# HAHHHD/mllp

Hardware: AMD Instinct MI355X
Metric: LP instances/sec (fwd+bwd) on Netlib batch; achieved HBM GB/s on CSR SpMM (higher is better)
Workload: dtype f32; 1 GPU; netlib_full: BASELINE.json configs[2], 97 instances / 1,074,147 nnz per global batch, one block-diagonal batch per GPU, one Adam step per global batch: fwd + BCE + bwd + gradient all-reduce + Adam, fp32; global_batch=97, instances_rank0=97, nnz_rank0=1074147, hip_graph=False, parallelism=dp1

## Files before the change

mllp_amd/csrc/fused_kernels.hip:

```cpp
#include <algorithm>
#include <vector>

#include "device_utils.h"
#include "host_graph.h"
#include "internal.h"
#include "node_bodies.h"

namespace mllp {

typedef float f32x4m __attribute__((ext_vector_type(4)));

#ifdef MLLP_TIMING_BUILD
static int g_fused_abl = [] {
    const char* e = getenv("MLLP_FUSED_ABL");
    return e ? atoi(e) : 0;
}();
#define FUSED_ABL(bit) ((J.abl & (bit)) != 0)
__device__ unsigned long long g_fused_stamps[8192 * 8];
__device__ unsigned long long g_fused_stamps1[8192 * 8];
#define FUSED_STAMP(k)                                                                      \
    {                                                                                       \
        __builtin_amdgcn_sched_barrier(0);                                                  \
        const unsigned long long now_ = __builtin_amdgcn_s_memtime();                       \
        __builtin_amdgcn_sched_barrier(0);                                                  \
        stamp_sum[k] += now_ - stamp_last;                                                  \
        stamp_last = now_;                                                                  \
    }
#else
#define FUSED_ABL(bit) false
#define FUSED_STAMP(k)
#endif

constexpr int FT = 768;
constexpr int FW = FT / 64;
constexpr int RT = 1024;
constexpr int MAXJOBS = 2;

constexpr int NP = FUSED_NP;
static_assert(NP == FUSED_PARTS, "partition count");

struct PartTiers {
    int row0, n_block, n_wave, n_group, n_base;
};
struct ItemsDev {
    const int* __restrict__ sptr;
    const int2* __restrict__ sent;
    const float2* __restrict__ sax;
    int n_dst, nnz;
    const int* __restrict__ order;
    int nw, L;
    PartTiers part[NP];
};

static ItemsDev items_dev(const FusedOrient& o, int which) {
    const bool scalar = which == 1;
    ItemsDev d;
    d.order = which == 0 ? o.lst16 : which == 1 ? o.lst1 : o.lst16x2;
    d.nw = which == 0 ? o.nw16 : which == 1 ? o.nw1 : o.nw16x2;
    d.L = which == 0 ? o.L16 : which == 1 ? o.L1 : o.L16x2;
    d.sptr = o.sptr;
    d.sent = reinterpret_cast<const int2*>(o.sent);
    d.sax = reinterpret_cast<const float2*>(o.sax);
    d.n_dst = o.n_dst;
    d.nnz = o.nnz;
    for (int q = 0; q < NP; ++q) {
        const FusedTiersDev& t = scalar ? o.t1[q] : o.t16[q];
        d.part[q].row0 = o.row0[q];
        d.part[q].n_block = t.n_block; d.part[q].n_wave = t.n_wave; d.part[q].n_group = t.n_group; d.part[q].n_base = t.n_base;
    }
    return d;
}

constexpr int TS = 17;
constexpr int TILE = 16 * TS;
__device__ __forceinline__ void tile_put(float* tile, const float4& v, int lane) {
    float* d = tile + (lane >> 2) * TS + 4 * (lane & 3);
    d[0] = v.x; d[1] = v.y; d[2] = v.z; d[3] = v.w;
}
__device__ __forceinline__ float4 tile_get(const float* tile, int lane) {
    const float* d = tile + (lane >> 2) * TS + 4 * (lane & 3);
    return make_float4(d[0], d[1], d[2], d[3]);
}
__device__ __forceinline__ void tile_rows(const float* tile, int lane, float (&a)[4]) {
#pragma unroll
    for (int s = 0; s < 4; ++s) a[s] = tile[(lane & 15) * TS + 4 * s + (lane >> 4)];
}
__device__ __forceinline__ void tile_cols(const float* tile, int lane, float (&a)[4]) {
#pragma unroll
    for (int s = 0; s < 4; ++s) a[s] = tile[(4 * s + (lane >> 4)) * TS + (lane & 15)];
}
__device__ __forceinline__ void tile_put_result(float* tile, const f32x4m& d, int lane) {
#pragma unroll
    for (int j = 0; j < 4; ++j) tile[(4 * (lane >> 4) + j) * TS + (lane & 15)] = d[j];
}
struct MatB {
    float w[4];
};
__device__ __forceinline__ MatB matB(const float* __restrict__ W, int ld, int lane) {
    MatB b;
#pragma unroll
    for (int s = 0; s < 4; ++s) b.w[s] = W[(lane & 15) * ld + 4 * s + (lane >> 4)];
    return b;
}
__device__ __forceinline__ MatB matB_t(const float* __restrict__ W, int ld, int lane) {
    MatB b;
#pragma unroll
    for (int s = 0; s < 4; ++s) b.w[s] = W[(4 * s + (lane >> 4)) * ld + (lane & 15)];
    return b;
}
__device__ __forceinline__ void matB_store(float* lds, const MatB& b, int lane) {
    *reinterpret_cast<float4*>(lds + 4 * lane) = make_float4(b.w[0], b.w[1], b.w[2], b.w[3]);
}
__device__ __forceinline__ MatB matB_lds(const float* lds, int lane) {
    const float4 v = *reinterpret_cast<const float4*>(lds + 4 * lane);
    MatB b;
    b.w[0] = v.x; b.w[1] = v.y; b.w[2] = v.z; b.w[3] = v.w;
    return b;
}
__device__ __forceinline__ f32x4m mat_apply(const float (&a)[4], const MatB& b, f32x4m acc) {
// ... 646 lines not shown
            const float Sr = __shfl(S, row_l, 64), ur = __shfl(un, row_l, 64), zr = __shfl(zn, row_l, 64), xr = __shfl(x, row_l, 64);
            float4 v = lds4(W.bs + ch);
            fma4(Sr, lds4(W.bv + ch), v);
            fma4(ur, lds4(W.we + ch), v);
            fma4(zr, lds4(W.wv + ch), v);
            fma4(xr, lds4(W.ws + ch), v);
            if (row_l < n_valid)
                *reinterpret_cast<float4*>(J.h + (size_t)(base_row + row_l) * 16 + ch) =
                    make_float4(fmaxf(v.x, 0.0f), fmaxf(v.y, 0.0f), fmaxf(v.z, 0.0f), fmaxf(v.w, 0.0f));
        }
        if (r.writer) {
            J.Z[r.row] = zn;
            reinterpret_cast<float4*>(J.aux)[r.row] = make_float4(un, st.L > 0.0f ? st.m : 0.0f, rinv, S);
        }
        return;
    }
    if (!r.writer) return;
    float o[16];
#pragma unroll
    for (int c = 0; c < 16; ++c) {
        float v = W.bs[c];
        v = fmaf(S, W.bv[c], v);
        v = fmaf(un, W.we[c], v);
        v = fmaf(W.wv[c], zn, v);
        v = fmaf(W.ws[c], x, v);
        o[c] = fmaxf(v, 0.0f);
    }
    float4* hd = reinterpret_cast<float4*>(J.h + (size_t)r.row * 16);
    hd[0] = make_float4(o[0], o[1], o[2], o[3]);
    hd[1] = make_float4(o[4], o[5], o[6], o[7]);
    hd[2] = make_float4(o[8], o[9], o[10], o[11]);
    hd[3] = make_float4(o[12], o[13], o[14], o[15]);
    J.Z[r.row] = zn;
    reinterpret_cast<float4*>(J.aux)[r.row] = make_float4(un, st.L > 0.0f ? st.m : 0.0f, rinv, S);
}

__global__ __launch_bounds__(FT) void fused_fwd1_kernel(FwdLaunch1 A) {
    __shared__ FwdW1 Ws_[MAXJOBS];
    __shared__ float merge_lds[FW * 4];
    const int tid = threadIdx.x, lane = tid & 63;
    for (int j = 0; j < A.n_jobs; ++j) {
        const FwdJob1& J = A.job[j];
        FwdW1& W = Ws_[j];
        if (tid < 16) {
            W.wv[tid] = J.p.Wv[tid]; W.ws[tid] = J.p.Ws[tid];
            W.bv[tid] = J.p.bv[tid]; W.we[tid] = J.p.we[tid]; W.bs[tid] = J.p.bs[tid];
        }
        if (tid == 0) {
            W.pq = J.D[OFF_PQ]; W.pq0 = J.D[OFF_PQ0]; W.pt = J.D[OFF_PT]; W.pt0 = J.D[OFF_PT0];
        }
    }
    __syncthreads();
    const BlockPart B = block_part();
    for (int j = 0; j < A.n_jobs; ++j) {
        const FwdJob1& J = A.job[j];
        const PartTiers P = J.s.part[B.px];
        for (int k = B.bi; k < P.n_block; k += B.gp)
            fwd1_row(J, Ws_[j], block_slot<1>(J.s, P.row0 + k, tid), lane, merge_lds);
        WaveList wl = wave_list(J.s, B.px, B.gw);
        for (int c0 = 0; c0 < wl.L; c0 += 64) {
            wave_list_chunk(wl, c0, lane);
            int it = wave_list_get(wl, 0);
            SlotReq q = item_request<1>(J.s, P, max(it, 0), lane);
            for (int k = 0; it >= 0; ++k) {
                const int itn = wave_list_get(wl, k + 1);
                const RowSlot r = slot_make(q);
                q = item_request<1>(J.s, P, max(itn, 0), lane);
                fwd1_row(J, Ws_[j], r, lane, merge_lds);
                it = itn;
            }
        }
    }
}

struct BwdJob16 {
    ItemsDev s;
    const float* __restrict__ x_src;
    const float* __restrict__ x_dst;
    const float* __restrict__ D;
    ConvParams p;
    const float* __restrict__ h;
    const float* __restrict__ dh_a;
    const float* __restrict__ dh_b;
    const float* __restrict__ Z;
    const float* __restrict__ aux;
    float* __restrict__ rec;
    float* __restrict__ dx_dst;
    int mask_dx;
    float* __restrict__ stats;
#ifdef MLLP_TIMING_BUILD
    int abl;
#endif
};
struct BwdLaunch16 {
    BwdJob16 job[MAXJOBS];
    int n_jobs;
};
struct BwdW16 {
    float BWvT[256], BPq[256], BWsT[256], BPqT[256];
    float pq0[16], Pt[16], Pb[16], bv[16], we[16];
    float pt0;
};
struct BwdState {
    float4 dq;
    float ds, dt;
};

__device__ __forceinline__ void bwd16_step(const Gather4& g, int k0, int n_mine, const float4& qp, const float4& gv, float t,
                                           float m, float rinv, float ge, float cc, BwdState& st) {
#define MLLP_BWD_SLOT(K, A_, X_)                                                           \
    {                                                                                      \
        const float l_ = fmaf(A_, t, quad_sum(dot4(qp, X_)));                              \
        const float al_ = (k0 + K < n_mine) ? exp_acc(l_ - m) * rinv : 0.0f;               \
        const float dl_ = al_ * (quad_sum(dot4(gv, X_)) + fmaf(A_, ge, cc));               \
        st.ds += dl_;                                                                      \
        st.dt = fmaf(dl_, A_, st.dt);                                                      \
        fma4(dl_, X_, st.dq);                                                              \
    }
    MLLP_BWD_SLOT(0, g.a0, g.x0)
    MLLP_BWD_SLOT(1, g.a1, g.x1)
    MLLP_BWD_SLOT(2, g.a2, g.x2)
    MLLP_BWD_SLOT(3, g.a3, g.x3)
#undef MLLP_BWD_SLOT
}

// ... 317 lines not shown
    if (!dst16_merge<1>(bs, r.mode, merge_lds, tiles, lane, part)) return;
    dst16_dx(W, tiles, bs, r, JJ.dx_dst, true, xpos, part, lane);
    StatCols c;
    dst16_stat_cols(tiles, bs, r, false, part, lane, c);
    stats_accumulate(c, acc, park, lane);
}

__global__ __launch_bounds__(FT) void fused_l3_kernel(L3Job JJ) {
    __shared__ L3W W;
    __shared__ float merge_lds[FW * 20];
    __shared__ float head_lds[FW * 18];
    __shared__ float tiles_[FW * TB_N * TILE];
    __shared__ __attribute__((aligned(16))) float park_[FW * L3_PARK];
    const int tid = threadIdx.x, lane = tid & 63, wave = tid >> 6, part = lane & 3;
    const FwdJob16& J = JJ.f;
    stage_weights<true, true>(W, J.D, J.p, J.fcw, J.fcb, tid);
    __syncthreads();
    float* tiles = tiles_ + wave * TB_N * TILE;
    HeadAcc ha;
    ha.w = f4zero(); ha.b = 0.0f; ha.l = 0.0f;
    float* park = park_ + wave * L3_PARK;
    f32x4m acc[L3_REG_TILES];
#pragma unroll
    for (int i = 0; i < L3_REG_TILES; ++i) acc[i] = splat4(0.0f);
#pragma unroll
    for (int i = L3_REG_TILES; i < STAT_TILES; ++i) park_put(park, i - L3_REG_TILES, lane, splat4(0.0f));
    const BlockPart B = block_part();
    const PartTiers P = J.s.part[B.px];
    walk_two_deep(J, P, B, tid, [&](const RowSlot& r, const float4& xd, int2& en, int lrow, const SlotReq& q1, int it2,
                                    FwdNext& nx) __attribute__((always_inline)) {
        l3_row(JJ, W, P, r, xd, en, lrow, q1, it2, nx, part, lane, merge_lds, tiles, park, ha, acc);
    });
    __syncthreads();
#pragma unroll
    for (int i = 0; i < STAT_TILES; ++i) {
        const f32x4m a = i < L3_REG_TILES ? acc[min(i, L3_REG_TILES - 1)] : park_get(park, max(i - L3_REG_TILES, 0), lane);
        stats_tile_store(a, i, tiles_, JJ.stats, tid);
    }
    head_partials_store<FW>(ha, head_lds, J.head_part, tid);
}

struct SrcJob16 {
    ItemsDev s;
    const float* __restrict__ x;
    const float* __restrict__ rec;
    float* __restrict__ dx;
    const float* __restrict__ addp;
    float addw;
    int mask;
};
struct SrcLaunch16 {
    SrcJob16 job[MAXJOBS];
    int n_jobs;
};

__device__ __forceinline__ void src16_row(const SrcJob16& J, const RowSlot& r, float4& xj_io, int2& en, const SlotReq& qn,
                                          RowSlot& rn, int part, int lane, float* merge_lds) {
    const int n_mine = slot_count(r);
    const float4 xj = xj_io;
    const float4 addv = ld4(J.addp + (size_t)max(r.row, 0) * 16 + 4 * part);
    float4 acc = f4zero();
    for (int k0 = 0; __any(k0 < n_mine); k0 += 2) {
        const int colm = en.x;
        const float am = __int_as_float(en.y);
        const int c0 = quad_bcast_i<0>(colm), c1 = quad_bcast_i<1>(colm);
        const float a0 = quad_bcast<0>(am), a1 = quad_bcast<1>(am);
        const bool ok0 = k0 < n_mine, ok1 = k0 + 1 < n_mine;
        const float* rr0 = J.rec + (size_t)c0 * REC_W;
        const float* rr1 = J.rec + (size_t)c1 * REC_W;
        const float4 q0 = ld4(rr0 + 4 * part), g0 = ld4(rr0 + 16 + 4 * part), s0 = ld4(rr0 + 32);
        const float cc0 = rr0[36];
        const float4 q1 = ld4(rr1 + 4 * part), g1 = ld4(rr1 + 16 + 4 * part), s1 = ld4(rr1 + 32);
        const float cc1 = rr1[36];
        const int kn = k0 + 2 + (part & 1);
        en = kn < n_mine ? J.s.sent[r.first + kn * r.stride] : make_int2(0, 0);
        {
            const float l = fmaf(a0, s0.x, quad_sum(dot4(q0, xj)));
            const float al = ok0 ? exp_acc(l - s0.y) * s0.z : 0.0f;
            const float dl = al * (quad_sum(dot4(g0, xj)) + fmaf(a0, s0.w, cc0));
            fma4(al, g0, acc);
            fma4(dl, q0, acc);
        }
        {
            const float l = fmaf(a1, s1.x, quad_sum(dot4(q1, xj)));
            const float al = ok1 ? exp_acc(l - s1.y) * s1.z : 0.0f;
            const float dl = al * (quad_sum(dot4(g1, xj)) + fmaf(a1, s1.w, cc1));
            fma4(al, g1, acc);
            fma4(dl, q1, acc);
        }
    }
    rn = slot_make(qn);
    xj_io = rn.row >= 0 ? ld4(J.x + (size_t)rn.row * 16 + 4 * part) : f4zero();
    en = first_entries<2>(J.s, rn, part);
    if (r.mode >= 1) {
        acc.x = shared_sum4(acc.x, r.mode); acc.y = shared_sum4(acc.y, r.mode);
        acc.z = shared_sum4(acc.z, r.mode); acc.w = shared_sum4(acc.w, r.mode);
    }
    if (r.mode == 3) {
        const int wave = threadIdx.x >> 6;
        if (lane < 4) *reinterpret_cast<float4*>(merge_lds + wave * 20 + 4 * part) = acc;
        __syncthreads();
        float4 v = f4zero();
        for (int w = 0; w < FW; ++w) v = f4add(v, lds4(merge_lds + w * 20 + 4 * part));
        acc = v;
        __syncthreads();
    }
    fma4(J.addw, addv, acc);
    if (J.mask) {
        if (!(xj.x > 0.0f)) acc.x = 0.0f;
        if (!(xj.y > 0.0f)) acc.y = 0.0f;
        if (!(xj.z > 0.0f)) acc.z = 0.0f;
        if (!(xj.w > 0.0f)) acc.w = 0.0f;
    }
    if (r.writer) *reinterpret_cast<float4*>(J.dx + (size_t)r.row * 16 + 4 * part) = acc;
}

__global__ __launch_bounds__(FT) void fused_src16_kernel(SrcLaunch16 A) {
    __shared__ float merge_lds[FW * 20];
    const int tid = threadIdx.x, lane = tid & 63, part = lane & 3;
    const BlockPart B = block_part();
    for (int j = 0; j < A.n_jobs; ++j) {
        const SrcJob16& J = A.job[j];
        const PartTiers P = J.s.part[B.px];
        const RowSlot none = empty_slot();
        for (int k = B.bi; k < P.n_block; k += B.gp) {
            const RowSlot r = block_slot<4>(J.s, P.row0 + k, tid);
            float4 xj = ld4(J.x + (size_t)r.row * 16 + 4 * part);
            int2 en = first_entries<2>(J.s, r, part);
            RowSlot rn;
            src16_row(J, r, xj, en, empty_request(), rn, part, lane, merge_lds);
        }
        WaveList wl = wave_list(J.s, B.px, B.gw);
        for (int c0 = 0; c0 < wl.L; c0 += 64) {
            wave_list_chunk(wl, c0, lane);
            int it = wave_list_get(wl, 0);
            RowSlot r = it >= 0 ? item_slot<4>(J.s, P, it, lane) : none;
            float4 xj = r.row >= 0 ? ld4(J.x + (size_t)r.row * 16 + 4 * part) : f4zero();
            int2 en = first_entries<2>(J.s, r, part);
            for (int k = 0; it >= 0; ++k) {
                const int itn = wave_list_get(wl, k + 1);
                const SlotReq qn = itn >= 0 ? item_request<4>(J.s, P, itn, lane) : empty_request();
                RowSlot rn;
                src16_row(J, r, xj, en, qn, rn, part, lane, merge_lds);
                r = rn;
                it = itn;
            }
        }
    }
}

struct BwdJob1 {
    ItemsDev s;
    const float* __restrict__ x_dst;
    const float* __restrict__ D;
    ConvParams p;
    const float* __restrict__ g;
    const float* __restrict__ Z;
    const float* __restrict__ aux;
    float* __restrict__ stats;
};
struct BwdLaunch1 {
    BwdJob1 job[MAXJOBS];
    int n_jobs;
};
struct alignas(16) BwdW1 {
    float wv[16], bv[16], we[16];
    float pq, pq0, pt, pt0;
};
constexpr int G1S = 17, R1S = 9;
constexpr int TILE1 = 64 * G1S + 64 * R1S;

__device__ __forceinline__ void bwd1_row(const BwdJob1& J, const BwdW1& W, const RowSlot& r, int lane, float* merge_lds,
                                         float* tiles, f32x4m& accT, float (&accS)[6]
#ifdef MLLP_TIMING_BUILD
                                         , unsigned long long (&stamp_sum)[8], unsigned long long& stamp_last
#endif
) {
    FUSED_STAMP(0)
    const bool writer = r.writer;
    Ent8 E;
    ent8_load(J.s, r, 0, E);
    const int rowc = max(r.row, 0);
    float gv = 0.0f, ge = 0.0f, gb = 0.0f;
    if (r.mode == 0) {
        const int base_row = __builtin_amdgcn_readfirstlane(r.row);
        const int n_valid = __popcll(__ballot(r.row >= 0));
        float* gt = tiles;
        float* rt = tiles + 64 * G1S;
#pragma unroll
        for (int q = 0; q < 4; ++q) {
            const int idx = lane + 64 * q, row_l = idx >> 2, ch = (idx & 3) * 4;
            const size_t ro = (size_t)min(base_row + row_l, J.s.n_dst - 1) * 16 + ch;
            const float4 a = ld4(J.g + ro);
            const bool on = row_l < n_valid;
            const float4 g = make_float4(on ? a.x : 0.0f, on ? a.y : 0.0f, on ? a.z : 0.0f, on ? a.w : 0.0f);
            const float pv = quad_sum(dot4(g, lds4(W.wv + ch))), pe = quad_sum(dot4(g, lds4(W.we + ch)));
            const float pb = quad_sum(dot4(g, lds4(W.bv + ch)));
            float* d = gt + row_l * G1S + ch;
            d[0] = g.x; d[1] = g.y; d[2] = g.z; d[3] = g.w;
            if ((lane & 3) == 0) { rt[row_l * R1S + 5] = pv; rt[row_l * R1S + 6] = pe; rt[row_l * R1S + 7] = pb; }
        }
// ... 288 lines not shown
    return ok_s != 0;
}
__global__ __launch_bounds__(RT) void fused_tail_kernel(TailArgs A, int n_conv) {
    const unsigned long long G = gridDim.x, epoch = A.sync[1];
    const int b = blockIdx.x;
    const float step = A.state[0] + 1.0f, lr = A.state[1], b1 = A.state[2], b2 = A.state[3];
    fused_reduce_body(A.R, n_conv);
    if (!tail_barrier(A.sync, (epoch + 1) * G, A.err)) return;
    if (b < n_conv) {
        finalize_conv_body(A.cin[b], A.p[b], A.R.out[b], 1, A.grads[b]);
        __syncthreads();
        const int off = (int)(A.grads[b] - A.grads_all), n = 4 * FEAT * A.cin[b] + 5 * FEAT;
        adam_slice(A.params + off, A.grads_all + off, A.m + off, A.v + off, step, lr, b1, b2, A.eps, 1.0f, n);
        __syncthreads();
        if (threadIdx.x < BLOCK) param_prep_body(A.p[b], A.cin[b], A.D[b]);
    } else if (b == n_conv) {
        for (int k = threadIdx.x; k < A.n_zero; k += RT) A.zero[k] = 0.0f;
        const int off = (int)(A.R.head_out - A.grads_all);
        adam_slice(A.params + off, A.grads_all + off, A.m + off, A.v + off, step, lr, b1, b2, A.eps, 1.0f, A.n_params - off);
        if (threadIdx.x == 0) {
            A.state[0] = step;
            A.sync[1] = epoch + 1;
        }
    }
}

__global__ __launch_bounds__(256) void fused_fill_kernel(int n_dst, const int* __restrict__ perm, const int* __restrict__ ptr,
                                                         const int* __restrict__ idx, const float* __restrict__ val,
                                                         const int* __restrict__ inv_src, const int* __restrict__ sptr,
                                                         int2* __restrict__ sent) {
    const int k = blockIdx.x * 4 + (threadIdx.x >> 6), lane = threadIdx.x & 63;
    if (k >= n_dst) return;
    const int r = perm[k], beg = ptr[r], deg = ptr[r + 1] - beg, o = sptr[k];
    for (int e = lane; e < deg; e += 64) sent[o + e] = make_int2(inv_src[idx[beg + e]], __float_as_int(val[beg + e]));
}
__global__ void fused_permute_kernel(int n, const int* __restrict__ perm, const float* __restrict__ src, float* __restrict__ dst) {
    for (int i = blockIdx.x * blockDim.x + threadIdx.x; i < n; i += gridDim.x * blockDim.x) dst[i] = src[perm[i]];
}
__global__ void fused_pregather_kernel(int64_t nnz, const int2* __restrict__ sent, const float* __restrict__ xs,
                                       float2* __restrict__ sax) {
    for (int64_t e = blockIdx.x * (int64_t)blockDim.x + threadIdx.x; e < nnz; e += (int64_t)gridDim.x * blockDim.x) {
        const int2 v = sent[e];
        sax[e] = make_float2(__int_as_float(v.y), xs[v.x]);
    }
}

#ifdef MLLP_TIMING_BUILD
extern "C" int mllp_timing_read_stamps(unsigned long long* host, int n) {
    return hipMemcpyFromSymbol(host, HIP_SYMBOL(g_fused_stamps), (size_t)n * sizeof(unsigned long long)) == hipSuccess ? 0 : -1;
}
extern "C" int mllp_timing_read_stamps1(unsigned long long* host, int n) {
    return hipMemcpyFromSymbol(host, HIP_SYMBOL(g_fused_stamps1), (size_t)n * sizeof(unsigned long long)) == hipSuccess ? 0 : -1;
}
#endif

template <class T>
static int dev_alloc(mllp_graph* g, size_t count, T** out, const T* host = nullptr, size_t room = 1) {
    void* p = nullptr;
    MLLP_HIP_TRY(hipMalloc(&p, std::max<size_t>(count, room) * sizeof(T)));
    if (count < room) MLLP_HIP_TRY(hipMemset(p, 0, room * sizeof(T)));
    g->allocs.push_back(p);
    if (host && count) MLLP_HIP_TRY(hipMemcpy(p, host, count * sizeof(T), hipMemcpyHostToDevice));
    *out = static_cast<T*>(p);
    return MLLP_OK;
}

static void set_tiers(FusedTiersDev& d, const FusedTiers& t) {
    d.n_block = t.n_block; d.n_wave = t.n_wave; d.n_group = t.n_group; d.n_base = t.n_base;
}

int fused_refill_values(mllp_graph* g, hipStream_t s) {
    int rc;
    if (g->M > 0) {
        hipLaunchKernelGGL(fused_fill_kernel, dim3((unsigned)((g->M + 3) / 4)), dim3(256), 0, s, (int)g->M, g->perm_c, g->A.ptr,
                           g->A.idx, g->A.val, g->inv_v, g->FA.sptr, reinterpret_cast<int2*>(g->FA.sent));
        if ((rc = check_launch("fused_fill A"))) return rc;
    }
    if (g->N > 0) {
        hipLaunchKernelGGL(fused_fill_kernel, dim3((unsigned)((g->N + 3) / 4)), dim3(256), 0, s, (int)g->N, g->perm_v, g->At.ptr,
                           g->At.idx, g->At.val, g->inv_c, g->FAt.sptr, reinterpret_cast<int2*>(g->FAt.sent));
        if ((rc = check_launch("fused_fill At"))) return rc;
    }
    return MLLP_OK;
}

int fused_graph_build(mllp_graph* g, const int* h_csr_ptr, const int* h_csc_ptr) {
    if (g->fused_built) return MLLP_OK;
    if ((int64_t)g->h_csr_ptr.size() != g->M + 1 && !h_csr_ptr) return fail(MLLP_EINVAL, "fused path: no host row pointers");
    HostFusedOrient hc, hv;
    {
#ifdef MLLP_SCALAR_PARTITION
        const std::vector<int> part = host_partition_instances(host_instance_cost(h_csr_ptr, g->h_inst_ptr_m),
                                                               host_instance_cost(h_csc_ptr, g->h_inst_ptr_n), FUSED_PARTS);
#else
        const std::vector<int> part = host_partition_instances_v(host_instance_loads(h_csr_ptr, g->h_inst_ptr_m),
                                                                 host_instance_loads(h_csc_ptr, g->h_inst_ptr_n), FUSED_PARTS);
#endif
        host_build_fused_orient(h_csr_ptr, (int)g->M, g->h_inst_ptr_m, part, &hc);
        host_build_fused_orient(h_csc_ptr, (int)g->N, g->h_inst_ptr_n, part, &hv);
    }
    int rc;
    if ((rc = dev_alloc(g, (size_t)g->M, &g->perm_c, hc.perm.data()))) return rc;
    if ((rc = dev_alloc(g, (size_t)g->N, &g->perm_v, hv.perm.data()))) return rc;
    if ((rc = dev_alloc(g, (size_t)g->M, &g->inv_c, hc.inv.data()))) return rc;
    if ((rc = dev_alloc(g, (size_t)g->N, &g->inv_v, hv.inv.data()))) return rc;
    FusedOrient& A = g->FA;
    FusedOrient& At = g->FAt;
    A.n_dst = (int)g->M; A.n_src = (int)g->N; A.nnz = (int)g->nnz;
    At.n_dst = (int)g->N; At.n_src = (int)g->M; At.nnz = (int)g->nnz;
    for (int q = 0; q < NP; ++q) {
        set_tiers(A.t16[q], hc.t16[q]); set_tiers(A.t1[q], hc.t1[q]);
        set_tiers(At.t16[q], hv.t16[q]); set_tiers(At.t1[q], hv.t1[q]);
    }
    for (int q = 0; q <= NP; ++q) { A.row0[q] = hc.row0[q]; At.row0[q] = hv.row0[q]; }
    {
        const int gp = fused_grid(g) / NP;
        const HostFusedOrient* ho[2] = {&hc, &hv};
        FusedOrient* dv[2] = {&A, &At};
        for (int k = 0; k < 2; ++k) {
            HostWaveLists l16, l16x2, l1;
            host_build_wave_lists(*ho[k], false, gp * FW, FW, 4, &l16);
            host_build_wave_lists(*ho[k], false, 2 * gp * FW, FW, 2, &l16x2);
            host_build_wave_lists(*ho[k], true, gp * FW, FW, 8, &l1);
            FusedOrient& d = *dv[k];
            d.L16 = l16.L; d.nw16 = l16.waves_per_part;
            d.L16x2 = l16x2.L; d.nw16x2 = l16x2.waves_per_part;
            d.L1 = l1.L; d.nw1 = l1.waves_per_part;
            if ((rc = dev_alloc(g, l16.order.size(), &d.lst16, l16.order.data()))) return rc;
            if ((rc = dev_alloc(g, l16x2.order.size(), &d.lst16x2, l16x2.order.data()))) return rc;
            if ((rc = dev_alloc(g, l1.order.size(), &d.lst1, l1.order.data()))) return rc;
        }
    }
    if ((rc = dev_alloc(g, (size_t)g->M + 1, &A.sptr, hc.sptr.data(), 2))) return rc;
    if ((rc = dev_alloc(g, (size_t)g->N + 1, &At.sptr, hv.sptr.data(), 2))) return rc;
    if ((rc = dev_alloc(g, (size_t)g->nnz * 2, &A.sent, (const int*)nullptr, 2))) return rc;
    if ((rc = dev_alloc(g, (size_t)g->nnz * 2, &At.sent, (const int*)nullptr, 2))) return rc;
    if ((rc = dev_alloc(g, (size_t)g->nnz * 2, &A.sax, (const float*)nullptr, 2))) return rc;
    if ((rc = dev_alloc(g, (size_t)g->nnz * 2, &At.sax, (const float*)nullptr, 2))) return rc;
    if ((rc = dev_alloc(g, (size_t)g->N, &g->inv_n_p))) return rc;
    if ((rc = dev_alloc(g, (size_t)g->N, &g->x1_p))) return rc;
    if ((rc = dev_alloc(g, (size_t)g->M, &g->x2_p))) return rc;
    if ((rc = dev_alloc(g, (size_t)g->N, &g->labels_p))) return rc;
    if (!g->tail_sync) {
        if ((rc = dev_alloc(g, (size_t)4, &g->tail_sync))) return rc;
        MLLP_HIP_TRY(hipMemset(g->tail_sync, 0, 32));
        MLLP_HIP_TRY(hipHostMalloc((void**)&g->tail_err_host, 64, hipHostMallocMapped));
        *g->tail_err_host = 0u;
        MLLP_HIP_TRY(hipHostGetDevicePointer((void**)&g->tail_err_dev, g->tail_err_host, 0));
    }
    if ((rc = fused_refill_values(g, 0))) return rc;
    if (g->N > 0) {
        hipLaunchKernelGGL(fused_permute_kernel, dim3(256), dim3(256), 0, 0, (int)g->N, g->perm_v, g->inv_n, g->inv_n_p);
        if ((rc = check_launch("fused_permute inv_n"))) return rc;
    }
    MLLP_HIP_TRY(hipDeviceSynchronize());
    g->fused_built = true;
    return MLLP_OK;
}

int fused_bind(mllp_graph* g, const float* x1, const float* x2, const float* labels, hipStream_t s) {
    int rc;
    hipStreamCaptureStatus cap = hipStreamCaptureStatusNone;
    (void)hipStreamIsCapturing(s, &cap);
    const bool capturing = cap != hipStreamCaptureStatusNone;
    if (capturing) g->bind_captured = true;
    if (g->bind_captured) g->bound_x1 = g->bound_x2 = g->bound_labels = nullptr;
    if (x1 != g->bound_x1 || x2 != g->bound_x2) {
        if (g->N > 0) hipLaunchKernelGGL(fused_permute_kernel, dim3(256), dim3(256), 0, s, (int)g->N, g->perm_v, x1, g->x1_p);
        if (g->M > 0) hipLaunchKernelGGL(fused_permute_kernel, dim3(256), dim3(256), 0, s, (int)g->M, g->perm_c, x2, g->x2_p);
        if (g->nnz > 0) {
            hipLaunchKernelGGL(fused_pregather_kernel, dim3(1024), dim3(256), 0, s, g->nnz,
                               reinterpret_cast<const int2*>(g->FA.sent), g->x1_p, reinterpret_cast<float2*>(g->FA.sax));
            hipLaunchKernelGGL(fused_pregather_kernel, dim3(1024), dim3(256), 0, s, g->nnz,
                               reinterpret_cast<const int2*>(g->FAt.sent), g->x2_p, reinterpret_cast<float2*>(g->FAt.sax));
        }
// ... 88 lines not shown
    BwdJob16 J = {};
    J.s = items_dev(o, 0);
    J.x_src = x_src; J.x_dst = x_dst; J.D = w.derived; J.p = conv_params_at(conv_at(m.P, c), MODEL_CONV[c].cin);
    J.h = h; J.dh_a = dh_a; J.dh_b = dh_b; J.Z = w.Z; J.aux = w.aux;
    J.rec = need_rec ? w.rec : nullptr;
    J.dx_dst = dx_dst;
    J.mask_dx = mask_dx ? 1 : 0;
    J.stats = w.stats;
#ifdef MLLP_TIMING_BUILD
    J.abl = g_fused_abl;
#endif
    return J;
}
static SrcJob16 src_job16(const FusedOrient& o_src_major, const ConvWs& w, const float* x_rows, float* dx, const float* add) {
    SrcJob16 J = {};
    J.s = items_dev(o_src_major, 2);
    J.x = x_rows; J.rec = w.rec; J.dx = dx;
    J.addp = add ? add : x_rows; J.addw = add ? 1.0f : 0.0f; J.mask = 1;
    return J;
}
static BwdJob1 bwd_job1(const FusedOrient& o, const FusedModel& m, int c, const float* x_dst, const float* g_masked) {
    const ConvWs& w = m.w.c[c];
    BwdJob1 J = {};
    J.s = items_dev(o, 1);
    J.x_dst = x_dst; J.D = w.derived; J.p = conv_params_at(conv_at(m.P, c), MODEL_CONV[c].cin);
    J.g = g_masked; J.Z = w.Z; J.aux = w.aux; J.stats = w.stats;
    return J;
}

int fused_backward(const mllp_graph* g, const FusedModel& m, bool premasked, float* grads, float* loss, hipStream_t s,
                   const FusedAdam* adam) {
    const int G = fused_grid(g);
    const ModelWs& w = m.w;
    int rc;
    const FusedOrient& A = g->FA;
    const FusedOrient& At = g->FAt;
    if (premasked) {
        L3Job L = {};
        L.f = l3_fwd_job(g, m, 2);
        L.rec = w.c[CONV_3V].rec; L.dx_dst = w.d2v; L.stats = w.c[CONV_3V].stats;
        hipLaunchKernelGGL(fused_l3_kernel, dim3(G), dim3(FT), 0, s, L);
        if ((rc = check_launch("fused_l3"))) return rc;
    } else {
        BwdLaunch16 L = {};
        L.n_jobs = 1;
        L.job[0] = bwd_job16(At, m, CONV_3V, w.h2c, w.h2v, w.h3v, w.d3v, nullptr, w.d2v, true, true);
        hipLaunchKernelGGL(fused_bwd16_kernel, dim3(G), dim3(FT), 0, s, L);
        if ((rc = check_launch("fused_bwd16 C3"))) return rc;
    }
    {
        SrcLaunch16 S = {};
        S.n_jobs = 1;
        S.job[0] = src_job16(A, w.c[CONV_3V], w.h2c, w.d2c, nullptr);
        hipLaunchKernelGGL(fused_src16_kernel, dim3(2 * G), dim3(FT), 0, s, S);
        if ((rc = check_launch("fused_src16 C3"))) return rc;
        BwdLaunch16 L = {};
        L.n_jobs = 1;
        L.job[0] = bwd_job16(At, m, CONV_2V, w.h1c, w.h1v, nullptr, w.d2v, nullptr, w.d1v, true, true);
        hipLaunchKernelGGL(fused_bwd16_kernel, dim3(G), dim3(FT), 0, s, L);
        if ((rc = check_launch("fused_bwd16 C2V"))) return rc;
    }
    {
        BwdLaunch16 L = {};
        L.n_jobs = 1;
        L.job[0] = bwd_job16(A, m, CONV_2C, w.h1v, w.h1c, nullptr, w.d2c, nullptr, w.d1c, true, true);
        hipLaunchKernelGGL(fused_bwd16_kernel, dim3(G), dim3(FT), 0, s, L);
        if ((rc = check_launch("fused_bwd16 C2C"))) return rc;
        SrcLaunch16 S = {};
        S.n_jobs = 2;
        S.job[0] = src_job16(A, w.c[CONV_2V], w.h1c, w.d1c_b, w.d1c);
        S.job[1] = src_job16(At, w.c[CONV_2C], w.h1v, w.d1v_b, w.d1v);
        hipLaunchKernelGGL(fused_src16_kernel, dim3(2 * G), dim3(FT), 0, s, S);
        if ((rc = check_launch("fused_src16 C2V + C2C"))) return rc;
    }
    {
        BwdLaunch1 L = {};
        L.n_jobs = 2;
        L.job[0] = bwd_job1(A, m, CONV_1C, g->x2_p, w.d1c_b);
        L.job[1] = bwd_job1(At, m, CONV_1V, g->x1_p, w.d1v_b);
        hipLaunchKernelGGL(fused_bwd1_kernel, dim3(G), dim3(FT), 0, s, L);
        if ((rc = check_launch("fused_bwd1"))) return rc;
    }
    ReduceArgs R = {};
    for (int c = 0; c < MODEL_CONVS; ++c) { R.stats[c] = w.c[c].stats; R.out[c] = w.c[c].red; }
    R.nblk = G;
    R.head_part = w.head_partials;
    R.head_out = grads + OFF_FC;
    R.loss_out = loss;
    if (adam) {
        TailArgs T = {};
        T.R = R;
        for (int c = 0; c < MODEL_CONVS; ++c) {
            T.p[c] = conv_params_at(conv_at(m.P, c), MODEL_CONV[c].cin);
            T.cin[c] = MODEL_CONV[c].cin;
            T.grads[c] = conv_at(grads, c);
            T.D[c] = w.c[c].derived;
        }
        T.zero = grads + OFF_UNUSED;
        T.n_zero = LEN_UNUSED;
        T.params = adam->params; T.grads_all = grads; T.m = adam->m; T.v = adam->v; T.state = adam->state;
        T.eps = adam->eps;
        T.n_params = adam->n;
        T.sync = g->tail_sync;
        T.err = g->tail_err_dev;
        if (g->tail_err_host && *(volatile unsigned*)g->tail_err_host != 0u)
            return fail(MLLP_EHIP, "the grid barrier of fused_tail_kernel timed out in an earlier step (the device was shared with "
                                   "other work): parameters and optimizer state since then are invalid; recreate the graph");
        hipLaunchKernelGGL(fused_tail_kernel, dim3(MODEL_CONVS * STAT_TILES + 1), dim3(RT), 0, s, T, MODEL_CONVS);
        return check_launch("fused_tail");
    }
    {
        hipLaunchKernelGGL(fused_reduce_kernel, dim3(MODEL_CONVS * STAT_TILES + 1), dim3(RT), 0, s, R, MODEL_CONVS);
        if ((rc = check_launch("fused_reduce"))) return rc;
    }
    return model_finalize(g, m.P, w, true, grads, s);
}

}
```

mllp_amd/csrc/host_graph.cpp:

```cpp
#include "host_graph.h"

#include <array>

#include <algorithm>
#include <atomic>
#include <thread>

#include "../../include/mllp_hip.h"

namespace mllp {

int host_build_batch(int64_t n_inst, const int64_t* inst_m, const int64_t* inst_n, const int64_t* indptr,
                     const int32_t* indices, const double* values, HostBatch* out, std::string* err,
                     unsigned max_threads) {
    auto bad_arg = [&](int code, const char* msg) {
        if (err) *err = msg;
        return code;
    };
    if (!out) return bad_arg(MLLP_EINVAL, "host_build_batch: out is null");
    if (n_inst < 0 || (n_inst > 0 && (!inst_m || !inst_n || !indptr)))
        return bad_arg(MLLP_EINVAL, "mllp_graph_create_host: null instance arrays");
    std::vector<int64_t> pm(n_inst + 1, 0), pn(n_inst + 1, 0), pe(n_inst + 1, 0), pp(n_inst + 1, 0);
    for (int64_t k = 0; k < n_inst; ++k) {
        if (inst_m[k] < 0 || inst_n[k] < 0) return bad_arg(MLLP_EINVAL, "negative instance size");
// ... 268 lines not shown
    for (int i = 0; i < n; ++i) {
        ca[i] = cost_a[i] + 1;
        cb[i] = cost_b[i] + 1;
        sa += ca[i]; sb += cb[i];
    }
    std::vector<int> order((size_t)n), part((size_t)n, 0);
    for (int i = 0; i < n; ++i) order[i] = i;
    std::stable_sort(order.begin(), order.end(), [&](int a, int b) { return ca[a] + cb[a] > ca[b] + cb[b]; });
    std::vector<int64_t> la((size_t)n_parts, 0), lb((size_t)n_parts, 0);
    for (int i : order) {
        int best = 0;
        double best_v = 0.0;
        for (int q = 0; q < n_parts; ++q) {
            const double v = std::max((double)(la[q] + ca[i]) / (double)sa, (double)(lb[q] + cb[i]) / (double)sb);
            if (q == 0 || v < best_v) { best = q; best_v = v; }
        }
        part[i] = best;
        la[best] += ca[i];
        lb[best] += cb[i];
    }
    return part;
}

void host_build_fused_orient(const int* ptr, int n, const std::vector<int64_t>& inst_off, const std::vector<int>& inst_part,
                             HostFusedOrient* out) {
    HostFusedOrient& o = *out;
    o = HostFusedOrient();
    n = std::max(n, 0);
    o.perm.resize((size_t)n);
    o.inv.resize((size_t)n);
    o.sptr.assign((size_t)n + 1, 0);
    std::vector<int> node_part((size_t)n, 0);
    for (size_t k = 0; k + 1 < inst_off.size(); ++k)
        for (int64_t r = inst_off[k]; r < inst_off[k + 1] && r < n; ++r) node_part[(size_t)r] = inst_part[k];
    for (int r = 0; r < n; ++r) o.perm[r] = r;
    std::stable_sort(o.perm.begin(), o.perm.end(), [&](int a, int b) {
        if (node_part[a] != node_part[b]) return node_part[a] < node_part[b];
        return ptr[a + 1] - ptr[a] > ptr[b + 1] - ptr[b];
    });
    for (int q = 0; q <= FUSED_PARTS; ++q) o.row0[q] = 0;
    for (int k = 0; k < n; ++k) {
        const int r = o.perm[k], deg = ptr[r + 1] - ptr[r], q = node_part[r];
        o.inv[r] = k;
        o.sptr[k + 1] = o.sptr[k] + deg;
        o.row0[q + 1]++;
        for (int which = 0; which < 2; ++which) {
            const int(&T)[3] = which ? FUSED_T1 : FUSED_T16;
            FusedTiers& t = which ? o.t1[q] : o.t16[q];
            if (deg > T[2]) t.n_block++;
            else if (deg > T[1]) t.n_wave++;
            else if (deg > T[0]) t.n_group++;
            else t.n_base++;
        }
    }
    for (int q = 0; q < FUSED_PARTS; ++q) o.row0[q + 1] += o.row0[q];
}

void host_build_wave_lists(const HostFusedOrient& o, bool scalar, int waves_per_part, int waves_per_wg, int nnz_per_step,
                           HostWaveLists* out) {
    HostWaveLists& wl = *out;
    wl = HostWaveLists();
    const int nw = std::max(waves_per_part, 1), wpg = std::max(std::min(waves_per_wg, nw), 1), gp = std::max(nw / wpg, 1);
    wl.waves_per_part = nw;
    const int U = scalar ? 64 : 16, RG = U / 4;
    const int e_base = std::max(nnz_per_step, 1), e_group = 4 * e_base, e_wave = (scalar ? 64 : 16) * e_base;
    std::vector<std::vector<int>> lists((size_t)FUSED_PARTS * nw);
    for (int q = 0; q < FUSED_PARTS; ++q) {
        const FusedTiers& t = scalar ? o.t1[q] : o.t16[q];
        const int n_gitems = (t.n_group + RG - 1) / RG, n_bitems = (t.n_base + U - 1) / U;
        const int n_items = t.n_wave + n_gitems + n_bitems;
        auto deg_of = [&](int rl) { const int k = o.row0[q] + rl; return (int64_t)o.sptr[(size_t)k + 1] - o.sptr[(size_t)k]; };
        std::vector<std::pair<int64_t, int>> items((size_t)n_items);
        for (int it = 0; it < n_items; ++it) {
            int64_t steps;
            if (it < t.n_wave) steps = (deg_of(t.n_block + it) + e_wave - 1) / e_wave;
            else if (it < t.n_wave + n_gitems) steps = (deg_of(t.n_block + t.n_wave + (it - t.n_wave) * RG) + e_group - 1) / e_group;
            else steps = (deg_of(t.n_block + t.n_wave + t.n_group + (it - t.n_wave - n_gitems) * U) + e_base - 1) / e_base;
            items[(size_t)it] = {FUSED_COST_ITEM + FUSED_COST_STEP * std::max<int64_t>(steps, 1), it};
        }
        std::stable_sort(items.begin(), items.end(), [](const auto& a, const auto& b) { return a.first > b.first; });
        std::vector<int64_t> load((size_t)nw, 0), slow((size_t)nw, 0);
        for (int w = 0; w < nw; ++w) {
            const int bi = w / wpg;
            const int n_rows = bi < gp && t.n_block > bi ? (t.n_block - bi + gp - 1) / gp : 0;
            slow[(size_t)w] = 1000 + 95 * ((w % wpg) / 4);
            load[(size_t)w] = FUSED_COST_BLOCK_ROW * n_rows * slow[(size_t)w] / 1000;
        }
        for (const auto& itc : items) {
            int best = 0;
            int64_t best_t = 0;
            for (int w = 0; w < nw; ++w) {
                const int64_t tw = load[(size_t)w] + itc.first * slow[(size_t)w] / 1000;
                if (w == 0 || tw < best_t) { best = w; best_t = tw; }
            }
            lists[(size_t)q * nw + best].push_back(itc.second);
            load[(size_t)best] = best_t;
        }
        for (int w = 0; w < nw; ++w) {
            wl.max_load = std::max(wl.max_load, load[(size_t)w]);
            wl.sum_load += load[(size_t)w];
            wl.L = std::max(wl.L, (int)lists[(size_t)q * nw + w].size());
        }
    }
    wl.L = std::max(wl.L, 1);
    wl.order.assign((size_t)FUSED_PARTS * nw * wl.L, -1);
    for (size_t k = 0; k < lists.size(); ++k) std::copy(lists[k].begin(), lists[k].end(), wl.order.begin() + k * wl.L);
}

}
```

mllp_amd/csrc/host_graph.h:

```cpp
#pragma once
#include <stdint.h>

#include <string>
#include <vector>

namespace mllp {

struct HostBatch {
    int64_t M = 0, N = 0, nnz = 0, n_inst = 0;
    std::vector<int64_t> pm, pn;
    std::vector<int> csr_ptr, csr_idx;
    std::vector<float> csr_val;
    std::vector<int> csc_ptr, csc_idx;
    std::vector<float> csc_val;
};

int host_build_batch(int64_t n_inst, const int64_t* inst_m, const int64_t* inst_n, const int64_t* indptr,
                     const int32_t* indices, const double* values, HostBatch* out, std::string* err,
                     unsigned max_threads = 0);

struct TierConfig {
    int tier_wave = 0, tier_block = 0, chunk_nnz = 0;
};
TierConfig host_choose_tiers(int64_t nnz, int tier_wave, int tier_block);

struct HostTiers {
    std::vector<int> rows_wave;
    std::vector<int> chunks;
    std::vector<int> split;
    int n_group = 0, n_slots = 0;
    bool short_rows = false;
};
void host_build_tiers(const int* ptr, int n_dst, const TierConfig& cfg, HostTiers* out);

constexpr int FUSED_PARTS = 8;
struct FusedTiers {
    int n_block = 0, n_wave = 0, n_group = 0, n_base = 0;
};
struct HostFusedOrient {
    std::vector<int> perm;
    std::vector<int> inv;
    std::vector<int> sptr;
    int row0[FUSED_PARTS + 1];
    FusedTiers t16[FUSED_PARTS], t1[FUSED_PARTS];
};
constexpr int FUSED_T16[3] = {16, 64, 1024};
constexpr int FUSED_T1[3] = {16, 64, 4096};
constexpr int64_t FUSED_COST_ITEM = 5300, FUSED_COST_STEP = 2000, FUSED_COST_BLOCK_ROW = 25000;
std::vector<int64_t> host_instance_cost(const int* ptr, const std::vector<int64_t>& inst_off);
std::vector<int> host_partition_instances(const std::vector<int64_t>& cost_a, const std::vector<int64_t>& cost_b, int n_parts);
constexpr int FUSED_BLOCK_ROW_ITEMS = 10;
constexpr int FUSED_LOAD_DIMS = 6;
struct InstLoad {
    int64_t d[FUSED_LOAD_DIMS] = {0, 0, 0, 0, 0, 0};
};
std::vector<InstLoad> host_instance_loads(const int* ptr, const std::vector<int64_t>& inst_off);
std::vector<int> host_partition_instances_v(const std::vector<InstLoad>& a, const std::vector<InstLoad>& b, int n_parts);
double host_partition_imbalance(const std::vector<InstLoad>& a, const std::vector<InstLoad>& b, const std::vector<int>& part,
                                int n_parts);
void host_build_fused_orient(const int* ptr, int n, const std::vector<int64_t>& inst_off, const std::vector<int>& inst_part,
                             HostFusedOrient* out);
struct HostWaveLists {
    std::vector<int> order;
    int L = 0, waves_per_part = 0;
    int64_t max_load = 0, sum_load = 0;
};
void host_build_wave_lists(const HostFusedOrient& o, bool scalar, int waves_per_part, int waves_per_wg, int nnz_per_step,
                           HostWaveLists* out);

}
```

mllp_amd/csrc/internal.h:

```cpp
#pragma once
#include <hip/hip_runtime.h>
#include <stdint.h>

#include <algorithm>
#include <string>
#include <vector>

#include "../../include/mllp_hip.h"

namespace mllp {

constexpr int FEAT = 16;
constexpr int BLOCK = 256;
constexpr int REC_W = 40;
constexpr int STAT_TILES = 7;
constexpr int STAT_FLOATS = STAT_TILES * 256;
constexpr int STAT_BLOCKS_MAX = 256;

void set_error(const std::string& msg);
int fail(int code, const std::string& msg);
int hip_fail(hipError_t e, const char* what);

#define MLLP_HIP_TRY(expr)                                              \
    do {                                                                \
// ... 55 lines not shown
    int64_t nnz = 0;
    int* tile_row = nullptr;
    int* tile_blk = nullptr;
    int* tile_col = nullptr;
    int* rows = nullptr;
    int* whdr = nullptr;
    unsigned* offs = nullptr;
    float* vals = nullptr;
    int* vmap = nullptr;
    double build_seconds = 0.0;
};

struct CopyArray {
    void** p;
    int64_t bytes;
};
enum { SC_TILE_BLK, SC_BLK_ID, SC_ROWS, SC_ENT, SC_TILE_ROW, SC_HDR };
enum { LC_TILE_BLK, LC_TILE_COL, LC_ROWS, LC_OFFS, LC_TILE_ROW, LC_WHDR, LC_VALS };
enum { TL_TILE_BLK, TL_BLK_ID, TL_PTR2, TL_PERM, TL_ENT };
std::vector<CopyArray> stream_copy_arrays(StreamCopy& sc, int geom);
std::vector<CopyArray> lane_copy_arrays(LaneCopy& lc);
std::vector<CopyArray> tiled_arrays(Tiled& tl, int variant, int64_t nnz);
int copy_alloc(const CopyArray& a);
void copy_free(const std::vector<CopyArray>& arrays);

struct Orient {
    LaneCopy lane1;
    StreamCopy stream[4];
    Tiled tiled[TILED_VARIANTS];
    int n_dst = 0, n_src = 0;
    int* ptr = nullptr;
    int* idx = nullptr;
    float* val = nullptr;
    int* rows_group = nullptr;
    int* rows_wave = nullptr;
    int* chunks = nullptr;
    int* split = nullptr;
    int n_group = 0, n_wave = 0, n_chunk = 0, n_split = 0, n_slots = 0;
    float* scratch = nullptr;
    int tier_wave = 0;
    bool short_rows = false;
};
struct FusedTiersDev {
    int n_block = 0, n_wave = 0, n_group = 0, n_base = 0;
};
constexpr int FUSED_NP = 8;
struct FusedOrient {
    int n_dst = 0, n_src = 0, nnz = 0;
    int* sptr = nullptr;
    int* sent = nullptr;
    float* sax = nullptr;
    int row0[FUSED_NP + 1] = {};
    FusedTiersDev t16[FUSED_NP], t1[FUSED_NP];
    int* lst16 = nullptr; int* lst16x2 = nullptr; int* lst1 = nullptr;
    int L16 = 0, L16x2 = 0, L1 = 0, nw16 = 0, nw16x2 = 0, nw1 = 0;
};
constexpr int SCRATCH_NS = 20;

}

struct mllp_graph {
    int64_t M = 0, N = 0, nnz = 0, n_inst = 0;
    mllp::Orient A;
    mllp::Orient At;
    float* inv_n = nullptr;
    int* inst_ptr_n = nullptr;
    int* inst_ptr_m = nullptr;
    std::vector<int64_t> h_inst_ptr_n, h_inst_ptr_m;
    std::vector<int> h_csr_ptr, h_csc_ptr;
    int tier_wave = 0, tier_block = 0, chunk_nnz = 0;
    int max_inst_n = 0;
    int n_cu = 256;
    int n_cu_dev = 256;
    int64_t grid_limit = 0;
    int path = 0;
    bool fused_built = false;
    mllp::FusedOrient FA, FAt;
    int* perm_v = nullptr;
    int* perm_c = nullptr;
    int* inv_v = nullptr;
    int* inv_c = nullptr;
    float* inv_n_p = nullptr;
    unsigned long long* tail_sync = nullptr;
    unsigned* tail_err_host = nullptr;
    unsigned* tail_err_dev = nullptr;
    float* x1_p = nullptr;
    float* x2_p = nullptr;
    float* labels_p = nullptr;
    const void* bound_x1 = nullptr;
    const void* bound_x2 = nullptr;
    const void* bound_labels = nullptr;
    bool bind_captured = false;
    int ws_path = -1;
    const void* ws_ptr = nullptr;
    const void* ws_params = nullptr;
    const void* folded_ws = nullptr;
    const void* folded_params = nullptr;
    int* at_pos = nullptr;
    float* scale_buf = nullptr;
    float* norm_scale = nullptr;
    int* plant_ws = nullptr;
    hipStream_t aux = nullptr;
    hipEvent_t ev[16] = {};
    std::vector<void*> allocs;
};

// ... 227 lines not shown
```

Baseline: 316,300 instances/s.

## Give src16 kernel its own tier thresholds and step-aware wave list balancing

Adds a separate tier classification (t16s) for the src16 backward kernel. Rows with degree above 256, rather than 1024, are promoted to whole-block processing. The src16 wave lists are built with a cost model that charges block rows per inner step, using a lower per-row constant and no slow-wave factor. The goal is to reduce load imbalance and long-tail waves in the src16 kernel, at the cost of more block-level rows with per-block merge overhead. Timing-build-only stamp instrumentation is also added for the fwd1 and src16 kernels.

```diff
diff --git a/mllp_amd/csrc/fused_kernels.hip b/mllp_amd/csrc/fused_kernels.hip
--- a/mllp_amd/csrc/fused_kernels.hip
+++ b/mllp_amd/csrc/fused_kernels.hip
@@ -18,6 +18,10 @@
 #define FUSED_ABL(bit) ((J.abl & (bit)) != 0)
 __device__ unsigned long long g_fused_stamps[8192 * 8];
 __device__ unsigned long long g_fused_stamps1[8192 * 8];
+constexpr int SRC_STAMP_WAVES = 8192;
+__device__ unsigned long long g_fused_stamps_src[2 * SRC_STAMP_WAVES * 8];
+__device__ unsigned long long g_fused_stamps_src_t[2 * SRC_STAMP_WAVES * 2];
+__device__ unsigned long long g_fused_stamps_f1[8192 * 8];
 #define FUSED_STAMP(k)                                                                      \
     {                                                                                       \
         __builtin_amdgcn_sched_barrier(0);                                                  \
@@ -64,7 +68,7 @@
     d.n_dst = o.n_dst;
     d.nnz = o.nnz;
     for (int q = 0; q < NP; ++q) {
-        const FusedTiersDev& t = scalar ? o.t1[q] : o.t16[q];
+        const FusedTiersDev& t = scalar ? o.t1[q] : which == 2 ? o.t16s[q] : o.t16[q];
         d.part[q].row0 = o.row0[q];
         d.part[q].n_block = t.n_block; d.part[q].n_wave = t.n_wave; d.part[q].n_group = t.n_group; d.part[q].n_base = t.n_base;
     }
@@ -817,11 +821,21 @@
     }
     __syncthreads();
     const BlockPart B = block_part();
+#ifdef MLLP_TIMING_BUILD
+    unsigned long long stamp_sum[8] = {0, 0, 0, 0, 0, 0, 0, 0};
+    unsigned long long stamp_last = __builtin_amdgcn_s_memtime();
+    const unsigned long long stamp_begin = stamp_last;
+#endif
     for (int j = 0; j < A.n_jobs; ++j) {
         const FwdJob1& J = A.job[j];
         const PartTiers P = J.s.part[B.px];
-        for (int k = B.bi; k < P.n_block; k += B.gp)
+        for (int k = B.bi; k < P.n_block; k += B.gp) {
             fwd1_row(J, Ws_[j], block_slot<1>(J.s, P.row0 + k, tid), lane, merge_lds);
+#ifdef MLLP_TIMING_BUILD
+            stamp_sum[5] += 1;
+#endif
+        }
+        FUSED_STAMP(1)
         WaveList wl = wave_list(J.s, B.px, B.gw);
         for (int c0 = 0; c0 < wl.L; c0 += 64) {
             wave_list_chunk(wl, c0, lane);
@@ -832,10 +846,21 @@
                 const RowSlot r = slot_make(q);
                 q = item_request<1>(J.s, P, max(itn, 0), lane);
                 fwd1_row(J, Ws_[j], r, lane, merge_lds);
+#ifdef MLLP_TIMING_BUILD
+                stamp_sum[7] += 1;
+#endif
                 it = itn;
             }
         }
-    }
+        FUSED_STAMP(0)
+    }
+#ifdef MLLP_TIMING_BUILD
+    if (lane == 0 && blockIdx.x * FW + (tid >> 6) < 8192) {
+        stamp_sum[6] = __builtin_amdgcn_s_memtime() - stamp_begin;
+        unsigned long long* d = g_fused_stamps_f1 + (size_t)(blockIdx.x * FW + (tid >> 6)) * 8;
+        for (int k = 0; k < 8; ++k) d[k] = stamp_sum[k];
+    }
+#endif
 }
 
 struct BwdJob16 {
@@ -1259,15 +1284,26 @@
 struct SrcLaunch16 {
     SrcJob16 job[MAXJOBS];
     int n_jobs;
+#ifdef MLLP_TIMING_BUILD
+    int stamp_slot;
+#endif
 };
 
 __device__ __forceinline__ void src16_row(const SrcJob16& J, const RowSlot& r, float4& xj_io, int2& en, const SlotReq& qn,
-                                          RowSlot& rn, int part, int lane, float* merge_lds) {
+                                          RowSlot& rn, int part, int lane, float* merge_lds
+#ifdef MLLP_TIMING_BUILD
+                                          , bool block_row, unsigned long long (&stamp_sum)[8], unsigned long long& stamp_last
+#endif
+) {
+    FUSED_STAMP(block_row ? 3 : 0)
     const int n_mine = slot_count(r);
     const float4 xj = xj_io;
     const float4 addv = ld4(J.addp + (size_t)max(r.row, 0) * 16 + 4 * part);
     float4 acc = f4zero();
     for (int k0 = 0; __any(k0 < n_mine); k0 += 2) {
+#ifdef MLLP_TIMING_BUILD
+        if (!block_row) stamp_sum[4] += 1;
+#endif
         const int colm = en.x;
         const float am = __int_as_float(en.y);
         const int c0 = quad_bcast_i<0>(colm), c1 = quad_bcast_i<1>(colm);
@@ -1296,6 +1332,7 @@
             fma4(dl, q1, acc);
         }
     }
+    FUSED_STAMP(block_row ? 3 : 1)
     rn = slot_make(qn);
     xj_io = rn.row >= 0 ? ld4(J.x + (size_t)rn.row * 16 + 4 * part) : f4zero();
     en = first_entries<2>(J.s, rn, part);
@@ -1320,12 +1357,21 @@
         if (!(xj.w > 0.0f)) acc.w = 0.0f;
     }
     if (r.writer) *reinterpret_cast<float4*>(J.dx + (size_t)r.row * 16 + 4 * part) = acc;
+    FUSED_STAMP(block_row ? 3 : 2)
 }
 
 __global__ __launch_bounds__(FT) void fused_src16_kernel(SrcLaunch16 A) {
     __shared__ float merge_lds[FW * 20];
     const int tid = threadIdx.x, lane = tid & 63, part = lane & 3;
     const BlockPart B = block_part();
+#ifdef MLLP_TIMING_BUILD
+    unsigned long long stamp_sum[8] = {0, 0, 0, 0, 0, 0, 0, 0};
+    unsigned long long stamp_last = __builtin_amdgcn_s_memtime();
+    const unsigned long long stamp_begin = stamp_last;
+#define STAMP_ARGS_SRC(block) , block, stamp_sum, stamp_last
+#else
+#define STAMP_ARGS_SRC(block)
+#endif
     for (int j = 0; j < A.n_jobs; ++j) {
         const SrcJob16& J = A.job[j];
         const PartTiers P = J.s.part[B.px];
@@ -1335,7 +1381,10 @@
             float4 xj = ld4(J.x + (size_t)r.row * 16 + 4 * part);
             int2 en = first_entries<2>(J.s, r, part);
             RowSlot rn;
-            src16_row(J, r, xj, en, empty_request(), rn, part, lane, merge_lds);
+            src16_row(J, r, xj, en, empty_request(), rn, part, lane, merge_lds STAMP_ARGS_SRC(true));
+#ifdef MLLP_TIMING_BUILD
+            stamp_sum[5] += 1;
+#endif
         }
         WaveList wl = wave_list(J.s, B.px, B.gw);
         for (int c0 = 0; c0 < wl.L; c0 += 64) {
@@ -1348,12 +1397,26 @@
                 const int itn = wave_list_get(wl, k + 1);
                 const SlotReq qn = itn >= 0 ? item_request<4>(J.s, P, itn, lane) : empty_request();
                 RowSlot rn;
-                src16_row(J, r, xj, en, qn, rn, part, lane, merge_lds);
+                src16_row(J, r, xj, en, qn, rn, part, lane, merge_lds STAMP_ARGS_SRC(false));
+#ifdef MLLP_TIMING_BUILD
+                stamp_sum[7] += 1;
+#endif
                 r = rn;
                 it = itn;
             }
         }
     }
+#undef STAMP_ARGS_SRC
+#ifdef MLLP_TIMING_BUILD
+    const int sw = blockIdx.x * FW + (tid >> 6);
+    if (lane == 0 && sw < SRC_STAMP_WAVES) {
+        stamp_sum[6] = __builtin_amdgcn_s_memtime() - stamp_begin;
+        unsigned long long* d = g_fused_stamps_src + ((size_t)(A.stamp_slot & 1) * SRC_STAMP_WAVES + sw) * 8;
+        for (int k = 0; k < 8; ++k) d[k] = stamp_sum[k];
+        unsigned long long* t = g_fused_stamps_src_t + ((size_t)(A.stamp_slot & 1) * SRC_STAMP_WAVES + sw) * 2;
+        t[0] = stamp_begin; t[1] = stamp_begin + stamp_sum[6];
+    }
+#endif
 }
 
 struct BwdJob1 {
@@ -1748,6 +1811,18 @@
 extern "C" int mllp_timing_read_stamps1(unsigned long long* host, int n) {
     return hipMemcpyFromSymbol(host, HIP_SYMBOL(g_fused_stamps1), (size_t)n * sizeof(unsigned long long)) == hipSuccess ? 0 : -1;
 }
+extern "C" int mllp_timing_read_stamps_f1(unsigned long long* host, int n) {
+    if (n < 0 || n > 8192 * 8) return -1;
+    return hipMemcpyFromSymbol(host, HIP_SYMBOL(g_fused_stamps_f1), (size_t)n * sizeof(unsigned long long)) == hipSuccess ? 0 : -1;
+}
+extern "C" int mllp_timing_read_stamps_src_t(unsigned long long* host, int n) {
+    if (n < 0 || n > 2 * SRC_STAMP_WAVES * 2) return -1;
+    return hipMemcpyFromSymbol(host, HIP_SYMBOL(g_fused_stamps_src_t), (size_t)n * sizeof(unsigned long long)) == hipSuccess ? 0 : -1;
+}
+extern "C" int mllp_timing_read_stamps_src(unsigned long long* host, int n) {
+    if (n < 0 || n > 2 * SRC_STAMP_WAVES * 8) return -1;
+    return hipMemcpyFromSymbol(host, HIP_SYMBOL(g_fused_stamps_src), (size_t)n * sizeof(unsigned long long)) == hipSuccess ? 0 : -1;
+}
 #endif
 
 template <class T>
@@ -1807,6 +1882,7 @@
     for (int q = 0; q < NP; ++q) {
         set_tiers(A.t16[q], hc.t16[q]); set_tiers(A.t1[q], hc.t1[q]);
         set_tiers(At.t16[q], hv.t16[q]); set_tiers(At.t1[q], hv.t1[q]);
+        set_tiers(A.t16s[q], hc.t16s[q]); set_tiers(At.t16s[q], hv.t16s[q]);
     }
     for (int q = 0; q <= NP; ++q) { A.row0[q] = hc.row0[q]; At.row0[q] = hv.row0[q]; }
     {
@@ -1816,7 +1892,7 @@
         for (int k = 0; k < 2; ++k) {
             HostWaveLists l16, l16x2, l1;
             host_build_wave_lists(*ho[k], false, gp * FW, FW, 4, &l16);
-            host_build_wave_lists(*ho[k], false, 2 * gp * FW, FW, 2, &l16x2);
+            host_build_src16_lists(*ho[k], 2 * gp * FW, FW, &l16x2);
             host_build_wave_lists(*ho[k], true, gp * FW, FW, 8, &l1);
             FusedOrient& d = *dv[k];
             d.L16 = l16.L; d.nw16 = l16.waves_per_part;
@@ -2011,6 +2087,9 @@
         SrcLaunch16 S = {};
         S.n_jobs = 1;
         S.job[0] = src_job16(A, w.c[CONV_3V], w.h2c, w.d2c, nullptr);
+#ifdef MLLP_TIMING_BUILD
+        S.stamp_slot = 0;
+#endif
         hipLaunchKernelGGL(fused_src16_kernel, dim3(2 * G), dim3(FT), 0, s, S);
         if ((rc = check_launch("fused_src16 C3"))) return rc;
         BwdLaunch16 L = {};
@@ -2029,6 +2108,9 @@
         S.n_jobs = 2;
         S.job[0] = src_job16(A, w.c[CONV_2V], w.h1c, w.d1c_b, w.d1c);
         S.job[1] = src_job16(At, w.c[CONV_2C], w.h1v, w.d1v_b, w.d1v);
+#ifdef MLLP_TIMING_BUILD
+        S.stamp_slot = 1;
+#endif
         hipLaunchKernelGGL(fused_src16_kernel, dim3(2 * G), dim3(FT), 0, s, S);
         if ((rc = check_launch("fused_src16 C2V + C2C"))) return rc;
     }
diff --git a/mllp_amd/csrc/host_graph.cpp b/mllp_amd/csrc/host_graph.cpp
--- a/mllp_amd/csrc/host_graph.cpp
+++ b/mllp_amd/csrc/host_graph.cpp
@@ -344,12 +344,18 @@
             else if (deg > T[0]) t.n_group++;
             else t.n_base++;
         }
+        FusedTiers& ts = o.t16s[q];
+        if (deg > FUSED_SRC16_WAVE_MAX) ts.n_block++;
+        else if (deg > FUSED_T16[1]) ts.n_wave++;
+        else if (deg > FUSED_T16[0]) ts.n_group++;
+        else ts.n_base++;
     }
     for (int q = 0; q < FUSED_PARTS; ++q) o.row0[q + 1] += o.row0[q];
 }
 
-void host_build_wave_lists(const HostFusedOrient& o, bool scalar, int waves_per_part, int waves_per_wg, int nnz_per_step,
-                           HostWaveLists* out) {
+namespace {
+void build_wave_lists(const HostFusedOrient& o, const FusedTiers (&tiers)[FUSED_PARTS], bool scalar, int waves_per_part,
+                      int waves_per_wg, int nnz_per_step, int64_t cost_block_row, int64_t cost_block_step, HostWaveLists* out) {
     HostWaveLists& wl = *out;
     wl = HostWaveLists();
     const int nw = std::max(waves_per_part, 1), wpg = std::max(std::min(waves_per_wg, nw), 1), gp = std::max(nw / wpg, 1);
@@ -358,7 +364,7 @@
     const int e_base = std::max(nnz_per_step, 1), e_group = 4 * e_base, e_wave = (scalar ? 64 : 16) * e_base;
     std::vector<std::vector<int>> lists((size_t)FUSED_PARTS * nw);
     for (int q = 0; q < FUSED_PARTS; ++q) {
-        const FusedTiers& t = scalar ? o.t1[q] : o.t16[q];
+        const FusedTiers& t = tiers[q];
         const int n_gitems = (t.n_group + RG - 1) / RG, n_bitems = (t.n_base + U - 1) / U;
         const int n_items = t.n_wave + n_gitems + n_bitems;
         auto deg_of = [&](int rl) { const int k = o.row0[q] + rl; return (int64_t)o.sptr[(size_t)k + 1] - o.sptr[(size_t)k]; };
@@ -375,8 +381,12 @@
         for (int w = 0; w < nw; ++w) {
             const int bi = w / wpg;
             const int n_rows = bi < gp && t.n_block > bi ? (t.n_block - bi + gp - 1) / gp : 0;
+            int64_t charge = cost_block_row * n_rows;
+            if (cost_block_step)
+                for (int k = bi; bi < gp && k < t.n_block; k += gp)
+                    charge += cost_block_step * ((deg_of(k) + (int64_t)wpg * e_wave - 1) / ((int64_t)wpg * e_wave));
             slow[(size_t)w] = 1000 + 95 * ((w % wpg) / 4);
-            load[(size_t)w] = FUSED_COST_BLOCK_ROW * n_rows * slow[(size_t)w] / 1000;
+            load[(size_t)w] = cost_block_step ? charge : charge * slow[(size_t)w] / 1000;
         }
         for (const auto& itc : items) {
             int best = 0;
@@ -398,5 +408,15 @@
     wl.order.assign((size_t)FUSED_PARTS * nw * wl.L, -1);
     for (size_t k = 0; k < lists.size(); ++k) std::copy(lists[k].begin(), lists[k].end(), wl.order.begin() + k * wl.L);
 }
-
-}
+}
+
+void host_build_wave_lists(const HostFusedOrient& o, bool scalar, int waves_per_part, int waves_per_wg, int nnz_per_step,
+                           HostWaveLists* out) {
+    build_wave_lists(o, scalar ? o.t1 : o.t16, scalar, waves_per_part, waves_per_wg, nnz_per_step, FUSED_COST_BLOCK_ROW, 0, out);
+}
+
+void host_build_src16_lists(const HostFusedOrient& o, int waves_per_part, int waves_per_wg, HostWaveLists* out) {
+    build_wave_lists(o, o.t16s, false, waves_per_part, waves_per_wg, 2, FUSED_SRC16_COST_BLOCK_ROW, FUSED_COST_STEP, out);
+}
+
+}
diff --git a/mllp_amd/csrc/host_graph.h b/mllp_amd/csrc/host_graph.h
--- a/mllp_amd/csrc/host_graph.h
+++ b/mllp_amd/csrc/host_graph.h
@@ -43,10 +43,13 @@
     std::vector<int> sptr;
     int row0[FUSED_PARTS + 1];
     FusedTiers t16[FUSED_PARTS], t1[FUSED_PARTS];
+    FusedTiers t16s[FUSED_PARTS];
 };
 constexpr int FUSED_T16[3] = {16, 64, 1024};
 constexpr int FUSED_T1[3] = {16, 64, 4096};
 constexpr int64_t FUSED_COST_ITEM = 5300, FUSED_COST_STEP = 2000, FUSED_COST_BLOCK_ROW = 25000;
+constexpr int FUSED_SRC16_WAVE_MAX = 256;
+constexpr int64_t FUSED_SRC16_COST_BLOCK_ROW = 5000;
 std::vector<int64_t> host_instance_cost(const int* ptr, const std::vector<int64_t>& inst_off);
 std::vector<int> host_partition_instances(const std::vector<int64_t>& cost_a, const std::vector<int64_t>& cost_b, int n_parts);
 constexpr int FUSED_BLOCK_ROW_ITEMS = 10;
@@ -67,5 +70,6 @@
 };
 void host_build_wave_lists(const HostFusedOrient& o, bool scalar, int waves_per_part, int waves_per_wg, int nnz_per_step,
                            HostWaveLists* out);
+void host_build_src16_lists(const HostFusedOrient& o, int waves_per_part, int waves_per_wg, HostWaveLists* out);
 
 }
diff --git a/mllp_amd/csrc/internal.h b/mllp_amd/csrc/internal.h
--- a/mllp_amd/csrc/internal.h
+++ b/mllp_amd/csrc/internal.h
@@ -131,6 +131,7 @@
     float* sax = nullptr;
     int row0[FUSED_NP + 1] = {};
     FusedTiersDev t16[FUSED_NP], t1[FUSED_NP];
+    FusedTiersDev t16s[FUSED_NP];
     int* lst16 = nullptr; int* lst16x2 = nullptr; int* lst1 = nullptr;
     int L16 = 0, L16x2 = 0, L1 = 0, nw16 = 0, nw16x2 = 0, nw1 = 0;
 };
```

After: 314,400 instances/s. Within noise of the previous version (-0.6%).
